# Ritesh622/Unbiased-Quantization-Distributed-Mean-Estimation

Measured on AMD Instinct MI355X. Metric: quantize+dequantize M-vectors/sec at d=2^20 (1/2/4/8 GPU) + NMSE vs reference, higher is better.
Workload: dtype f32

## Files before the change

unbiased-quantization-distributed-mean-estimation_amd/csrc/uq_unbiased_kernels.h:

```cpp

#ifndef UQ_UNBIASED_KERNELS_H
#define UQ_UNBIASED_KERNELS_H

#include "uq_common.h"

namespace {

constexpr int kQItems = 16;
constexpr int kQTile = kQBlock * kQItems;
constexpr int64_t kStreamMinClients = 256;
constexpr int64_t kSegMinTiles = 1024;

struct AbsOp {
    static constexpr bool kHist = false;
    float den, fm;
    uint32_t *h, *zn;
    __device__ static AbsOp make(const float*, float, int64_t) { return AbsOp{0.f, 0.f, nullptr, nullptr}; }
    __device__ float operator()(float v) const { return fabsf(v); }
    __device__ void apply4(const float (&v)[4], float (&a)[4]) const {
#pragma unroll
        for (int c = 0; c < 4; ++c) a[c] += fabsf(v[c]);
    }
};

// ... 1103 lines not shown
tile_out_kernel(const float* __restrict__ x, float* __restrict__ out, int8_t* __restrict__ codes,
                int32_t* __restrict__ overflow, int64_t d, int32_t tiles, float fm, const float* __restrict__ Xs,
                float Xval, const float* __restrict__ l1, const uint64_t* __restrict__ pre, int64_t ldo, int64_t ldc) {
    __shared__ __attribute__((aligned(16))) float s_x[kQTile];
    __shared__ float s_tab[kTab];
    __shared__ ScanLds sl;
    const int tid = threadIdx.x;
    const int32_t tile = blockIdx.x;
    const int64_t vec = blockIdx.y;
    TileRegs r;
    load_tile<VEC4>(r, x, d, tiles, (uint32_t)(vec * tiles + tile), tid);
    const float L = l1[vec];
    build_table(s_tab, tid, L, fm);
    stage_tile<VEC4>(r, s_x, tid);
    __syncthreads();
    const int64_t t0 = (int64_t)tile * kQTile;
    const int len = (int)((d - t0) < kQTile ? (d - t0) : kQTile);
    const DivPlan dp = div_plan(L);
    const double P = __longlong_as_double((long long)pre[vec * tiles + tile]);
    const Binade B = binade_of(P);
    TileState st;
    TileVals tv;
    if (len == kQTile)
        tile_pass1<true, true>(s_x, tv, sl, tid, len, dp, fm, B, st);
    else
        tile_pass1<false, true>(s_x, tv, sl, tid, len, dp, fm, B, st);
    double pnext;
    const double base = resolve_exact(P, B, st, tv, s_x, sl, tid, pnext);
    uint32_t cw[4];
    uint32_t kmax = 0u;
    tile_pass2<WQ, WC>(s_x, tv, s_tab, tid, base, L, fm, Xs ? Xs[vec] : Xval, cw, kmax);
    if (WC) {
        store_codes<CVEC>(codes + vec * ldc + t0, cw, len, tid);
        publish_kmax(kmax, L, overflow, vec, tid);
    }
    __syncthreads();
    if (WQ) store_tile<VEC4>(s_x, out + vec * ldo + t0, len, tid);
}

constexpr int kMeanThreads = 1024;
template <bool VEC4>
__global__ void __launch_bounds__(kMeanThreads)
client_mean_kernel(const float* __restrict__ q, int64_t n, int64_t d, int64_t ld, float n_div, int accumulate,
                   float* __restrict__ est) {
    const int64_t col = ((int64_t)blockIdx.x * blockDim.x + threadIdx.x) * 4;
    if (col >= d) return;
    if (VEC4) {
        float4 e = accumulate ? *reinterpret_cast<const float4*>(est + col) : make_float4(0.f, 0.f, 0.f, 0.f);
        int64_t j = 0;
        for (; j + 8 <= n; j += 8) {
            float4 t[8];
#pragma unroll
            for (int u = 0; u < 8; ++u) t[u] = ld_stream(reinterpret_cast<const float4*>(q + (j + u) * ld + col));
#pragma unroll
            for (int u = 0; u < 8; ++u) {
                e.x += t[u].x / n_div; e.y += t[u].y / n_div;
                e.z += t[u].z / n_div; e.w += t[u].w / n_div;
            }
        }
        for (; j < n; ++j) {
            const float4 t = *reinterpret_cast<const float4*>(q + j * ld + col);
            e.x += t.x / n_div; e.y += t.y / n_div; e.z += t.z / n_div; e.w += t.w / n_div;
        }
        *reinterpret_cast<float4*>(est + col) = e;
    } else {
        const int cnt = (int)((d - col) < 4 ? (d - col) : 4);
        for (int k = 0; k < cnt; ++k) {
            float e = accumulate ? est[col + k] : 0.f;
            for (int64_t j = 0; j < n; ++j) e += q[j * ld + col + k] / n_div;
            est[col + k] = e;
        }
    }
}

constexpr int kDecChunk = 4096;
constexpr int kMeanClients = 32;

__device__ __forceinline__ float decode_one(int8_t c, const float* tab) {
    const int ci = (int)c;
    const int k = ci ^ (ci >> 31);
    return __uint_as_float(__float_as_uint(tab[k]) ^ ((uint32_t)ci & 0x80000000u));
}

template <bool BIASED>
__device__ __forceinline__ float code_table_entry(float L, int k, float fm) {
    if constexpr (BIASED) return L * div1((float)k, div_plan_m(fm));
    else return (L * (float)k) / fm;
}

template <bool VEC, bool BIASED>
__device__ __forceinline__ void codes_decode_body(const int8_t* __restrict__ codes, const float* __restrict__ l1,
                                                  int64_t d, float fm, float* __restrict__ out) {
    __shared__ float tab[128];
    const int64_t vec = blockIdx.y;
    const int tid = threadIdx.x;
    const float L = l1[vec];
    if (tid < 128) tab[tid] = code_table_entry<BIASED>(L, tid, fm);
    __syncthreads();
    const int64_t i0 = (int64_t)blockIdx.x * kDecChunk + (int64_t)tid * 16;
    const int8_t* cr = codes + vec * d;
    float* orow = out + vec * d;
    if (VEC && i0 + 16 <= d) {
        const uint4 w = *reinterpret_cast<const uint4*>(cr + i0);
        const uint32_t ws[4] = {w.x, w.y, w.z, w.w};
#pragma unroll
        for (int k4 = 0; k4 < 4; ++k4) {
            float o[4];
#pragma unroll
            for (int c = 0; c < 4; ++c) o[c] = decode_one((int8_t)((ws[k4] >> (8 * c)) & 0xFF), tab);
            *reinterpret_cast<float4*>(orow + i0 + 4 * k4) = make_float4(o[0], o[1], o[2], o[3]);
        }
    } else {
        for (int64_t i = i0; i < i0 + 16 && i < d; ++i) orow[i] = decode_one(cr[i], tab);
    }
}

template <bool VEC>
__global__ void __launch_bounds__(256)
codes_decode_kernel(const int8_t* __restrict__ codes, const float* __restrict__ l1, int64_t d, float fm,
                    float* __restrict__ out) {
    codes_decode_body<VEC, false>(codes, l1, d, fm, out);
}

template <bool VEC>
__global__ void __launch_bounds__(256)
codes_decode_biased_kernel(const int8_t* __restrict__ codes, const float* __restrict__ l1, int64_t d, float fm,
                           float* __restrict__ out) {
    codes_decode_body<VEC, true>(codes, l1, d, fm, out);
}

constexpr int kMeanCpt = 8;
constexpr int kCodesMeanThreads = 512;
constexpr int kMeanUnroll = 16;
static_assert(kMeanClients == 2 * kMeanUnroll, "two code batches per table group");

__device__ __forceinline__ void mean_load_batch(uint2 (&w)[kMeanUnroll], const int8_t* cp, int64_t ldc) {
#pragma unroll
    for (int u = 0; u < kMeanUnroll; ++u) {
        const u32x2v t = __builtin_nontemporal_load(reinterpret_cast<const u32x2v*>(cp + (int64_t)u * ldc));
        w[u] = make_uint2(t.x, t.y);
    }
}

__device__ __forceinline__ void mean_add_batch(float (&e)[kMeanCpt], const uint2 (&w)[kMeanUnroll],
                                               const float (*tabn)[256], int jj) {
#pragma unroll
    for (int u = 0; u < kMeanUnroll; ++u) {
        const float* tb = tabn[jj + u];
#pragma unroll
        for (int k = 0; k < 4; ++k) e[k] += tb[(w[u].x >> (8 * k)) & 0xFF];
#pragma unroll
        for (int k = 0; k < 4; ++k) e[4 + k] += tb[(w[u].y >> (8 * k)) & 0xFF];
    }
}

template <bool BIASED = false>
__device__ __forceinline__ void mean_build_tables(float (*tabn)[256], const float* __restrict__ l1,
                                                  const int32_t* __restrict__ kmaxv, int64_t j0, int nb, int wid,
                                                  int lane, float fm, float n_div) {
    for (int jj = wid; jj < nb; jj += kCodesMeanThreads / kWave) {
        const float L = l1[j0 + jj];
        const int km = min(127, max(0, kmaxv[j0 + jj]));
        for (int k = lane; k <= km; k += kWave) {
            const float v = code_table_entry<BIASED>(L, k, fm) / n_div;
            tabn[jj][k] = v;
            tabn[jj][255 - k] = -v;
        }
    }
}

__device__ __forceinline__ void mean_add_bytes(float (&e)[kMeanCpt], const int8_t* __restrict__ codes, int64_t ldc,
                                               const float (*tabn)[256], int64_t j0, int nb, int64_t i0, int64_t d) {
    for (int jj = 0; jj < nb; ++jj)
        for (int k = 0; k < kMeanCpt; ++k)
            if (i0 + k < d) e[k] += tabn[jj][(uint8_t)codes[(j0 + jj) * ldc + i0 + k]];
}

__device__ __forceinline__ uint32_t mean_ovf_mask(const int32_t* __restrict__ kmaxv, int64_t j0, int nb) {
    uint32_t mk = 0;
    for (int jj = 0; jj < nb; ++jj) mk |= (kmaxv[j0 + jj] > 127 ? 1u : 0u) << jj;
    return mk;
}

__device__ __forceinline__ void mean_add_mixed(float (&e)[kMeanCpt], const int8_t* __restrict__ codes, int64_t ldc,
                                            const float* __restrict__ q, int64_t ldq, const float (*tabn)[256],
                                            uint32_t ovf, int64_t j0, int nb, int64_t i0, int64_t d, float n_div) {
    for (int jj = 0; jj < nb; ++jj) {
        const int64_t j = j0 + jj;
        if ((ovf >> jj) & 1u) {
            for (int k = 0; k < kMeanCpt; ++k)
                if (i0 + k < d) e[k] += q[j * ldq + i0 + k] / n_div;
        } else {
            for (int k = 0; k < kMeanCpt; ++k)
                if (i0 + k < d) e[k] += tabn[jj][(uint8_t)codes[j * ldc + i0 + k]];
        }
    }
}

template <bool VEC, bool ALL, bool BIASED>
__device__ __forceinline__ void codes_mean_body(const int8_t* __restrict__ codes, int64_t ldc,
                                                const float* __restrict__ l1, const int32_t* __restrict__ kmaxv,
                                                int64_t n, int64_t d, float fm, float n_div, int accumulate,
                                                float* __restrict__ est, const float* __restrict__ q, int64_t ldq) {
    __shared__ float tabn[kMeanClients][256];
    __shared__ uint32_t s_ovf;
    const int tid = threadIdx.x;
    const int lane = tid & (kWave - 1);
    const int wid = __builtin_amdgcn_readfirstlane(tid / kWave);
    const int64_t i0 = ((int64_t)blockIdx.x * kCodesMeanThreads + tid) * kMeanCpt;
    const bool full = ALL || (VEC && i0 + kMeanCpt <= d);
    float e[kMeanCpt];
#pragma unroll
    for (int k = 0; k < kMeanCpt; ++k) e[k] = (accumulate && i0 + k < d) ? est[i0 + k] : 0.0f;
    bool any = false;
    if (q) {
        if (tid == 0) s_ovf = 0u;
        __syncthreads();
        bool a = false;
        for (int64_t j = tid; j < n; j += kCodesMeanThreads) a = a || kmaxv[j] > 127;
        if (a) s_ovf = 1u;
        __syncthreads();
        any = s_ovf != 0u;
    }
    const int64_t groups = n / kMeanClients;
    if (any) {
        for (int64_t j0 = 0; j0 < n; j0 += kMeanClients) {
            const int nb = (int)min((int64_t)kMeanClients, n - j0);
            const uint32_t ovf = mean_ovf_mask(kmaxv, j0, nb);
            __syncthreads();
            mean_build_tables<BIASED>(tabn, l1, kmaxv, j0, nb, wid, lane, fm, n_div);
            __syncthreads();
            mean_add_mixed(e, codes, ldc, q, ldq, tabn, ovf, j0, nb, i0, d, n_div);
        }
    } else {
    const int8_t* cbase = codes + (full ? i0 : 0);
    uint2 wa[kMeanUnroll], wb[kMeanUnroll];
    if (VEC && groups > 0) mean_load_batch(wa, cbase, ldc);
    for (int64_t g = 0; g < groups; ++g) {
        const int64_t j0 = g * kMeanClients;
        __syncthreads();
        mean_build_tables<BIASED>(tabn, l1, kmaxv, j0, kMeanClients, wid, lane, fm, n_div);
        __syncthreads();
        if (VEC) {
            mean_load_batch(wb, cbase + (j0 + kMeanUnroll) * ldc, ldc);
            if (full) mean_add_batch(e, wa, tabn, 0);
            const int64_t jn = (j0 + kMeanClients + kMeanUnroll <= n) ? j0 + kMeanClients : n - kMeanUnroll;
            mean_load_batch(wa, cbase + jn * ldc, ldc);
            if (full) mean_add_batch(e, wb, tabn, kMeanUnroll);
        }
        if (!full) mean_add_bytes(e, codes, ldc, tabn, j0, kMeanClients, i0, d);
    }
    const int64_t jr = groups * kMeanClients;
    const int nr = (int)(n - jr);
    if (nr > 0) {
        __syncthreads();
        mean_build_tables<BIASED>(tabn, l1, kmaxv, jr, nr, wid, lane, fm, n_div);
        __syncthreads();
        if (full) {
            for (int jj = 0; jj < nr; ++jj) {
                const uint2 w = *reinterpret_cast<const uint2*>(codes + (jr + jj) * ldc + i0);
#pragma unroll
                for (int k = 0; k < 4; ++k) e[k] += tabn[jj][(w.x >> (8 * k)) & 0xFF];
#pragma unroll
                for (int k = 0; k < 4; ++k) e[4 + k] += tabn[jj][(w.y >> (8 * k)) & 0xFF];
            }
        } else {
            mean_add_bytes(e, codes, ldc, tabn, jr, nr, i0, d);
        }
    }
    }
    if (full) {
        *reinterpret_cast<float4*>(est + i0) = make_float4(e[0], e[1], e[2], e[3]);
        *reinterpret_cast<float4*>(est + i0 + 4) = make_float4(e[4], e[5], e[6], e[7]);
    } else {
        for (int k = 0; k < kMeanCpt; ++k)
            if (i0 + k < d) est[i0 + k] = e[k];
    }
}

template <bool VEC, bool ALL = false>
__global__ void __launch_bounds__(kCodesMeanThreads)
codes_mean_kernel(const int8_t* __restrict__ codes, int64_t ldc, const float* __restrict__ l1,
                  const int32_t* __restrict__ kmaxv, int64_t n, int64_t d, float fm, float n_div, int accumulate,
                  float* __restrict__ est, const float* __restrict__ q, int64_t ldq) {
    codes_mean_body<VEC, ALL, false>(codes, ldc, l1, kmaxv, n, d, fm, n_div, accumulate, est, q, ldq);
}

template <bool VEC, bool ALL = false>
__global__ void __launch_bounds__(kCodesMeanThreads)
codes_mean_biased_kernel(const int8_t* __restrict__ codes, int64_t ldc, const float* __restrict__ l1,
                         const int32_t* __restrict__ kmaxv, int64_t n, int64_t d, float fm, float n_div,
                         int accumulate, float* __restrict__ est, const float* __restrict__ q, int64_t ldq) {
    codes_mean_body<VEC, ALL, true>(codes, ldc, l1, kmaxv, n, d, fm, n_div, accumulate, est, q, ldq);
}

constexpr int kNibMax = 7;
constexpr int64_t kNibAlign = kCodesMeanThreads * kMeanCpt;

__device__ __forceinline__ void nib_load_batch(uint32_t (&w)[kMeanUnroll], const uint8_t* cp, int64_t ldn) {
#pragma unroll
    for (int u = 0; u < kMeanUnroll; ++u) w[u] = __builtin_nontemporal_load(reinterpret_cast<const uint32_t*>(cp + (int64_t)u * ldn));
}

__device__ __forceinline__ void nib_add_batch(float (&e)[kMeanCpt], const uint32_t (&w)[kMeanUnroll],
                                              const float (*tab)[16], int jj) {
#pragma unroll
    for (int u = 0; u < kMeanUnroll; ++u) {
        const float* tb = tab[jj + u];
#pragma unroll
        for (int k = 0; k < kMeanCpt; ++k) e[k] += tb[(w[u] >> (4 * k)) & 0xFu];
    }
}

constexpr int kNibChunk = 1024;
__device__ __forceinline__ void nib_build_tables(float (*tab)[16], const float* __restrict__ l1,
                                                 const int32_t* __restrict__ kmaxv, int64_t j0, int nb, float fm,
                                                 float n_div) {
    for (int e = threadIdx.x; e < nb * 8; e += kCodesMeanThreads) {
        const int jj = e >> 3, k = e & 7;
        const float L = l1[j0 + jj];
        const int km = min(kNibMax, max(0, kmaxv[j0 + jj]));
        if (k <= km) {
            const float v = ((L * (float)k) / fm) / n_div;
            tab[jj][k] = v;
            tab[jj][15 - k] = -v;
        }
    }
}

__global__ void __launch_bounds__(kCodesMeanThreads)
nibbles_mean_kernel(const uint8_t* __restrict__ nib, int64_t ldn, const float* __restrict__ l1,
                    const int32_t* __restrict__ kmaxv, int64_t n, int64_t d, float fm, float n_div, int accumulate,
                    float* __restrict__ est, const float* __restrict__ q, int64_t ldq) {
    __shared__ float tab[kNibChunk][16];
    __shared__ uint32_t s_ovf;
    const int tid = threadIdx.x;
    const int64_t i0 = ((int64_t)blockIdx.x * kCodesMeanThreads + tid) * kMeanCpt;
    float e[kMeanCpt];
    if (accumulate) {
        const float4 a = *reinterpret_cast<const float4*>(est + i0), b = *reinterpret_cast<const float4*>(est + i0 + 4);
        e[0] = a.x; e[1] = a.y; e[2] = a.z; e[3] = a.w; e[4] = b.x; e[5] = b.y; e[6] = b.z; e[7] = b.w;
    } else {
#pragma unroll
        for (int k = 0; k < kMeanCpt; ++k) e[k] = 0.0f;
    }
    if (tid == 0) s_ovf = 0u;
    __syncthreads();
    bool a = false;
    for (int64_t j = tid; j < n; j += kCodesMeanThreads) a = a || kmaxv[j] > kNibMax;
    if (a) s_ovf = 1u;
    __syncthreads();
    const bool any = s_ovf != 0u;
    const uint8_t* cbase = nib + i0 / 2;
    for (int64_t c0 = 0; c0 < n; c0 += kNibChunk) {
        const int nc = (int)min((int64_t)kNibChunk, n - c0);
        __syncthreads();
        nib_build_tables(tab, l1, kmaxv, c0, nc, fm, n_div);
        __syncthreads();
        const int full = any ? 0 : nc / kMeanClients * kMeanClients;
        if (full > 0) {
            uint32_t wa[kMeanUnroll], wb[kMeanUnroll];
            const uint8_t* cb = cbase + c0 * ldn;
            nib_load_batch(wa, cb, ldn);
            for (int g = 0; g < full; g += kMeanClients) {
                nib_load_batch(wb, cb + (int64_t)(g + kMeanUnroll) * ldn, ldn);
                nib_add_batch(e, wa, tab, g);
                const int gn = (g + kMeanClients + kMeanUnroll <= nc) ? g + kMeanClients : nc - kMeanUnroll;
                nib_load_batch(wa, cb + (int64_t)gn * ldn, ldn);
                nib_add_batch(e, wb, tab, g + kMeanUnroll);
            }
        }
        for (int jj = full; jj < nc; ++jj) {
            const int64_t j = c0 + jj;
            if (kmaxv[j] > kNibMax) {
                const float4 a4 = *reinterpret_cast<const float4*>(q + j * ldq + i0);
                const float4 b4 = *reinterpret_cast<const float4*>(q + j * ldq + i0 + 4);
                const float qq[kMeanCpt] = {a4.x, a4.y, a4.z, a4.w, b4.x, b4.y, b4.z, b4.w};
#pragma unroll
                for (int k = 0; k < kMeanCpt; ++k) e[k] += qq[k] / n_div;
            } else {
                const uint32_t w = *reinterpret_cast<const uint32_t*>(cbase + j * ldn);
#pragma unroll
                for (int k = 0; k < kMeanCpt; ++k) e[k] += tab[jj][(w >> (4 * k)) & 0xFu];
            }
        }
    }
    *reinterpret_cast<float4*>(est + i0) = make_float4(e[0], e[1], e[2], e[3]);
    *reinterpret_cast<float4*>(est + i0 + 4) = make_float4(e[4], e[5], e[6], e[7]);
}

}

#endif
```

Baseline: 0.4293.

## Use paired-nibble float2 lookup tables in LDS for nibble mean kernel

```diff
diff --git a/unbiased-quantization-distributed-mean-estimation_amd/csrc/uq_unbiased_kernels.h b/unbiased-quantization-distributed-mean-estimation_amd/csrc/uq_unbiased_kernels.h
--- a/unbiased-quantization-distributed-mean-estimation_amd/csrc/uq_unbiased_kernels.h
+++ b/unbiased-quantization-distributed-mean-estimation_amd/csrc/uq_unbiased_kernels.h
@@ -1429,13 +1429,57 @@
     for (int u = 0; u < kMeanUnroll; ++u) w[u] = __builtin_nontemporal_load(reinterpret_cast<const uint32_t*>(cp + (int64_t)u * ldn));
 }
 
+__device__ __forceinline__ uint32_t nib_pair_slot(uint32_t b) { return b ^ ((b >> 3) & 0x0Cu); }
+__device__ __forceinline__ uint32_t nib_pair_word(uint32_t w) { return w ^ ((w >> 3) & 0x0C0C0C0Cu); }
+
+template <int K>
+__device__ __forceinline__ uint32_t nib_byte_x8(uint32_t w) {
+    static_assert(K >= 0 && K < 4, "byte of a dword");
+    uint32_t r;
+    asm("v_lshlrev_b32_sdwa %0, %1, %2 dst_sel:DWORD dst_unused:UNUSED_PAD src0_sel:DWORD src1_sel:BYTE_%3"
+        : "=v"(r) : "v"(3u), "v"(w), "i"(K));
+    return r;
+}
+
+static_assert(kCodesMeanThreads == kMeanUnroll * 32, "one thread per (client, high nibble, half)");
+struct NibPairSrc {
+    float4 lo[2];
+    float vh;
+};
+__device__ __forceinline__ NibPairSrc nib_pair_load(const float (*tab)[16]) {
+    const int jj = threadIdx.x >> 5, hi = (threadIdx.x >> 1) & 15, half = threadIdx.x & 1;
+    NibPairSrc s;
+    s.lo[0] = *reinterpret_cast<const float4*>(&tab[jj][8 * half]);
+    s.lo[1] = *reinterpret_cast<const float4*>(&tab[jj][8 * half + 4]);
+    s.vh = tab[jj][hi];
+    return s;
+}
+__device__ __forceinline__ void nib_pair_store(float2 (*pair)[256], const NibPairSrc& s, int piece) {
+    const int jj = threadIdx.x >> 5, hi = (threadIdx.x >> 1) & 15, half = threadIdx.x & 1;
+    const int b = piece >> 1;
+    const int sw = (hi >> 1) & 3;
+    float4* dst = reinterpret_cast<float4*>(&pair[jj][hi * 16]) + 2 * ((2 * half + b) ^ sw) + (piece & 1);
+    *dst = (piece & 1) ? make_float4(s.lo[b].z, s.vh, s.lo[b].w, s.vh) : make_float4(s.lo[b].x, s.vh, s.lo[b].y, s.vh);
+}
+__device__ __forceinline__ void nib_build_pairs(float2 (*pair)[256], const float (*tab)[16]) {
+    const NibPairSrc s = nib_pair_load(tab);
+#pragma unroll
+    for (int piece = 0; piece < 4; ++piece) nib_pair_store(pair, s, piece);
+}
+
 __device__ __forceinline__ void nib_add_batch(float (&e)[kMeanCpt], const uint32_t (&w)[kMeanUnroll],
-                                              const float (*tab)[16], int jj) {
+                                              const float2 (*pair)[256], float2 (*next)[256], const NibPairSrc& src) {
 #pragma unroll
     for (int u = 0; u < kMeanUnroll; ++u) {
-        const float* tb = tab[jj + u];
-#pragma unroll
-        for (int k = 0; k < kMeanCpt; ++k) e[k] += tb[(w[u] >> (4 * k)) & 0xFu];
+        const char* tb = reinterpret_cast<const char*>(pair[u]);
+        const uint32_t s = nib_pair_word(w[u]);
+        const float2 v0 = *reinterpret_cast<const float2*>(tb + nib_byte_x8<0>(s));
+        const float2 v1 = *reinterpret_cast<const float2*>(tb + nib_byte_x8<1>(s));
+        const float2 v2 = *reinterpret_cast<const float2*>(tb + nib_byte_x8<2>(s));
+        const float2 v3 = *reinterpret_cast<const float2*>(tb + nib_byte_x8<3>(s));
+        e[0] += v0.x; e[1] += v0.y; e[2] += v1.x; e[3] += v1.y;
+        e[4] += v2.x; e[5] += v2.y; e[6] += v3.x; e[7] += v3.y;
+        if (u % 4 == 1) nib_pair_store(next, src, u / 4);
     }
 }
 
@@ -1455,14 +1499,25 @@
     }
 }
 
+static_assert(kNibChunk % kMeanClients == 0, "whole groups in every chunk but the last");
+struct NibLds {
+    float2 pair[2][kMeanUnroll][256];
+    float tab[kNibChunk][16];
+    uint32_t ovf;
+};
 __global__ void __launch_bounds__(kCodesMeanThreads)
 nibbles_mean_kernel(const uint8_t* __restrict__ nib, int64_t ldn, const float* __restrict__ l1,
                     const int32_t* __restrict__ kmaxv, int64_t n, int64_t d, float fm, float n_div, int accumulate,
                     float* __restrict__ est, const float* __restrict__ q, int64_t ldq) {
-    __shared__ float tab[kNibChunk][16];
-    __shared__ uint32_t s_ovf;
+    __shared__ alignas(16) NibLds lds;
+    float (*tab)[16] = lds.tab;
+    float2 (*pair)[kMeanUnroll][256] = lds.pair;
+    uint32_t& s_ovf = lds.ovf;
     const int tid = threadIdx.x;
     const int64_t i0 = ((int64_t)blockIdx.x * kCodesMeanThreads + tid) * kMeanCpt;
+    const uint8_t* cbase = nib + i0 / 2;
+    uint32_t wa[kMeanUnroll] = {}, wb[kMeanUnroll];
+    if (n >= kMeanClients) nib_load_batch(wa, cbase, ldn);
     float e[kMeanCpt];
     if (accumulate) {
         const float4 a = *reinterpret_cast<const float4*>(est + i0), b = *reinterpret_cast<const float4*>(est + i0 + 4);
@@ -1478,7 +1533,6 @@
     if (a) s_ovf = 1u;
     __syncthreads();
     const bool any = s_ovf != 0u;
-    const uint8_t* cbase = nib + i0 / 2;
     for (int64_t c0 = 0; c0 < n; c0 += kNibChunk) {
         const int nc = (int)min((int64_t)kNibChunk, n - c0);
         __syncthreads();
@@ -1486,15 +1540,19 @@
         __syncthreads();
         const int full = any ? 0 : nc / kMeanClients * kMeanClients;
         if (full > 0) {
-            uint32_t wa[kMeanUnroll], wb[kMeanUnroll];
+            nib_build_pairs(pair[0], tab);
+            __syncthreads();
             const uint8_t* cb = cbase + c0 * ldn;
-            nib_load_batch(wa, cb, ldn);
             for (int g = 0; g < full; g += kMeanClients) {
+                NibPairSrc src = nib_pair_load(tab + g + kMeanUnroll);
                 nib_load_batch(wb, cb + (int64_t)(g + kMeanUnroll) * ldn, ldn);
-                nib_add_batch(e, wa, tab, g);
-                const int gn = (g + kMeanClients + kMeanUnroll <= nc) ? g + kMeanClients : nc - kMeanUnroll;
-                nib_load_batch(wa, cb + (int64_t)gn * ldn, ldn);
-                nib_add_batch(e, wb, tab, g + kMeanUnroll);
+                nib_add_batch(e, wa, pair[0], pair[1], src);
+                __syncthreads();
+                src = nib_pair_load(tab + min(g + kMeanClients, kNibChunk - kMeanUnroll));
+                const int64_t jn = min(c0 + g + kMeanClients, n - kMeanUnroll);
+                nib_load_batch(wa, cbase + jn * ldn, ldn);
+                nib_add_batch(e, wb, pair[1], pair[0], src);
+                __syncthreads();
             }
         }
         for (int jj = full; jj < nc; ++jj) {
```

After: 0.4261. About the same (-0.7%).
